# JuliaGaussianProcesses/ApproximateGPs.jl

Measured on NVIDIA B200. Metric: SVGP ELBO+grad points/sec (FP64), higher is better.
Workload: dtype f64

## Files before the change

### approximategps.jl_b200/csrc/agp.cu

```cuda
#include <dlfcn.h>
#include <nccl.h>
#include <stdarg.h>
#include <stdio.h>
#include <string.h>

#include <algorithm>
#include <string>
#include <vector>

#include "../../include/agp.h"
#include "dense.cuh"
#include "f32sweep.cuh"
#include "gemm.cuh"
#include "kfun.cuh"
#include "laplace.cuh"
#include "sweep.cuh"

using namespace agp;

static thread_local std::string g_err;
static thread_local int32_t g_err_info = 0;
static int32_t fail(int32_t code, const char* fmt, ...) {
  char buf[1024];
  va_list ap;
// ... 87 lines not shown
  LikParams lp;
  std::vector<double> h_m;
};

enum { PC_TRSM_FWD = 0, PC_GEMM_BTA, PC_PERPOINT, PC_GEMM_BC, PC_TRSM_BWD, PC_SYRK, PC_KGRAD, PC_PREPARE, PC_FINISH, PC_ALLREDUCE, PC_LAPLACE, PC_F32_AUX, PC_COUNT };
static const char* const kProfNames[PC_COUNT] = {"trsm_kuf_fwd", "gemm_BtA", "perpoint", "gemm_BC", "trsm_bwd", "syrk_G", "kgrad",
                                                 "prepare_step", "finish_epilogue", "allreduce", "laplace", "f32_planes_gvec"};
struct ProfRec {
  int cls;
  cudaEvent_t a, b;
};
struct Prof {
  bool on = false;
  std::vector<cudaEvent_t> pool;
  size_t used = 0;
  std::vector<ProfRec> recs;
  double ms[PC_COUNT] = {0};
  int64_t cnt[PC_COUNT] = {0};
  cudaEvent_t get() {
    if (used == pool.size()) {
      cudaEvent_t e;
      cudaEventCreate(&e);
      pool.push_back(e);
    }
    return pool[used++];
  }
};

static void lap_release(agp_ctx* c);
static void chol_partition_release(agp_ctx* c);
struct agp_ctx {
  Prof prof;
  void* lap = nullptr;
  int device = 0;
  cudaStream_t stream = nullptr;
  cudaStream_t stream2 = nullptr;
  cudaEvent_t ev_trail = nullptr;
  cudaStream_t stream3 = nullptr;
  int part_state = 0;
  CUgreenCtx part_chain = nullptr, part_bulk = nullptr;
  cudaStream_t pstream_chain = nullptr, pstream_side = nullptr, pstream_trail = nullptr;
  cudaEvent_t ev_enter = nullptr, ev_leave = nullptr;
  int part_sms_chain = 0, part_sms_bulk = 0;
  cudaEvent_t ev_diag = nullptr, ev_prow = nullptr, ev_side = nullptr, ev_prio = nullptr;
  cudaStream_t stream_copy = nullptr;
  cudaEvent_t ev_copy = nullptr;
  int sms = 148;
  int64_t launches = 0;
  int64_t chunk_cols = 0;
  int nslab = 0, nsplit = 0;
  DevBuf z, zs, zn, zsp, mvec, mt, Lq, Kw, Lk, Lt, Ut, Bt_cm, Bt_rm, W1, W2, W3, W4, vec64, vec64b;
  DevBuf A, C, Ab, As, saa, sam, scc_part, dmu, dv, sc_part;
  DevBuf Kf, DKb;
  DevBuf gpart, Gpart, kpart, red, small, ghbuf;
  DevBuf qBt7, sBt7, sPm;
  DevBuf q6A, q6As, s6;
  DevBuf fA, fC, fAb, fAs, fBtc, fBtr, fLi;
  DevBuf qAb, sAb, qLi, sLi;
  DevBuf qK, sK, qLi7, sLi7, sxx_part;
  int* d_flags = nullptr;
  SvgpState st;
  ncclComm_t comm = nullptr;
  int nranks = 1, rank = 0;
  DevBuf mu_out, var_out, px1, px2, pxs1, pxn1, pxs2, pxn2, pcov;
};

struct agp_dataset {
  agp_ctx* ctx = nullptr;
  int64_t cap = 0, N = 0;
  int D = 0;
  double* X = nullptr;
  double* y = nullptr;
  DevBuf stage;
};

#define LAUNCHED(ctx) ((ctx)->launches++)
struct ProfScope {
  agp_ctx* c;
  bool on;
  ProfScope(agp_ctx* c_, int cls) : c(c_), on(c_->prof.on) {
    if (!on) return;
    ProfRec r{cls, c->prof.get(), c->prof.get()};
    cudaEventRecord(r.a, c->stream);
    c->prof.recs.push_back(r);
  }
  ~ProfScope() {
    if (on) cudaEventRecord(c->prof.recs.back().b, c->stream);
  }
};
#define KCHECK()                                                                                   \
  do {                                                                                             \
    cudaError_t e_ = cudaGetLastError();                                                           \
    if (e_ != cudaSuccess) return fail(AGP_ERR_CUDA, "kernel launch failed: %s (%s:%d)", cudaGetErrorString(e_), __FILE__, __LINE__); \
  } while (0)

extern "C" int32_t agp_ctx_create(int32_t device, agp_ctx** out) {
  if (!out) return fail(AGP_ERR_INVALID, "agp_ctx_create: out is NULL");
  int ndev = 0;
  cudaError_t e = cudaGetDeviceCount(&ndev);
  if (e != cudaSuccess || ndev == 0)
    return fail(AGP_ERR_CUDA, "no CUDA device available (%s); this library has no CPU fallback", cudaGetErrorString(e));
  if (device < 0 || device >= ndev) return fail(AGP_ERR_INVALID, "device %d out of range (0..%d)", device, ndev - 1);
  CU(cudaSetDevice(device));
  cudaDeviceProp prop;
  CU(cudaGetDeviceProperties(&prop, device));
  if (prop.major < 10)
    return fail(AGP_ERR_UNSUPPORTED, "device %s is sm_%d%d; this library is built for sm_100a only", prop.name, prop.major, prop.minor);
  agp_ctx* c = new agp_ctx();
  c->device = device;
  c->sms = prop.multiProcessorCount;
  int prio_lo = 0, prio_hi = 0;
  CU(cudaDeviceGetStreamPriorityRange(&prio_lo, &prio_hi));
  CU(cudaStreamCreateWithPriority(&c->stream, cudaStreamNonBlocking, prio_hi));
  CU(cudaStreamCreateWithPriority(&c->stream2, cudaStreamNonBlocking, prio_lo));
  CU(cudaStreamCreateWithPriority(&c->stream3, cudaStreamNonBlocking, prio_hi < prio_lo - 1 ? prio_hi + 1 : prio_hi));
  CU(cudaEventCreateWithFlags(&c->ev_trail, cudaEventDisableTiming));
  CU(cudaEventCreateWithFlags(&c->ev_diag, cudaEventDisableTiming));
  CU(cudaEventCreateWithFlags(&c->ev_prow, cudaEventDisableTiming));
  CU(cudaEventCreateWithFlags(&c->ev_side, cudaEventDisableTiming));
  CU(cudaEventCreateWithFlags(&c->ev_prio, cudaEventDisableTiming));
  CU(cudaStreamCreateWithFlags(&c->stream_copy, cudaStreamNonBlocking));
  CU(cudaEventCreateWithFlags(&c->ev_copy, cudaEventDisableTiming));
  CU(cudaMalloc(&c->d_flags, 4 * sizeof(int)));
  CU(cudaMemset(c->d_flags, 0, 4 * sizeof(int)));
  *out = c;
  return AGP_OK;
}

extern "C" int32_t agp_ctx_destroy(agp_ctx* c) {
  if (!c) return AGP_OK;
  cudaSetDevice(c->device);
  cudaStreamSynchronize(c->stream);
  if (c->comm && g_nccl.CommDestroy) g_nccl.CommDestroy(c->comm);
  DevBuf* bufs[] = {&c->z, &c->zs, &c->zn, &c->zsp, &c->mvec, &c->mt, &c->Lq, &c->Kw, &c->Lk, &c->Lt, &c->Ut, &c->Bt_cm, &c->Bt_rm,
                    &c->W1, &c->W2, &c->W3, &c->W4, &c->vec64, &c->vec64b, &c->A, &c->C, &c->Ab, &c->As, &c->Kf, &c->DKb, &c->saa, &c->sam,
                    &c->scc_part, &c->dmu, &c->dv, &c->sc_part, &c->gpart, &c->Gpart, &c->kpart, &c->red, &c->small, &c->ghbuf, &c->q6A, &c->q6As, &c->s6, &c->qBt7, &c->sBt7, &c->sPm, &c->fA, &c->fC, &c->fAb, &c->fAs, &c->fBtc, &c->fBtr, &c->fLi, &c->qAb, &c->sAb, &c->qLi, &c->sLi, &c->qK, &c->sK, &c->qLi7, &c->sLi7, &c->sxx_part,
                    &c->mu_out, &c->var_out, &c->px1, &c->px2, &c->pxs1, &c->pxn1, &c->pxs2, &c->pxn2, &c->pcov};
  for (DevBuf* b : bufs) b->release();
  lap_release(c);
  if (c->d_flags) cudaFree(c->d_flags);
  for (cudaEvent_t e : c->prof.pool) cudaEventDestroy(e);
  if (c->ev_trail) cudaEventDestroy(c->ev_trail);
  if (c->stream2) cudaStreamDestroy(c->stream2);
  for (cudaEvent_t e : {c->ev_diag, c->ev_prow, c->ev_side, c->ev_prio})
    if (e) cudaEventDestroy(e);
  if (c->stream3) cudaStreamDestroy(c->stream3);
  chol_partition_release(c);
  if (c->ev_copy) cudaEventDestroy(c->ev_copy);
  if (c->stream_copy) cudaStreamDestroy(c->stream_copy);
  cudaStreamDestroy(c->stream);
  delete c;
  return AGP_OK;
}

extern "C" int32_t agp_ctx_stream(agp_ctx* c, void** s) {
  if (!c || !s) return fail(AGP_ERR_INVALID, "agp_ctx_stream: NULL argument");
  *s = (void*)c->stream;
  return AGP_OK;
}
extern "C" int32_t agp_ctx_profile(agp_ctx* c, int32_t enable) {
  if (!c) return fail(AGP_ERR_INVALID, "agp_ctx_profile: NULL");
  c->prof.on = enable != 0;
  return AGP_OK;
}
extern "C" const char* agp_profile_class_name(int32_t cls) { return (cls >= 0 && cls < PC_COUNT) ? kProfNames[cls] : nullptr; }
extern "C" int32_t agp_ctx_profile_read(agp_ctx* c, int32_t max_classes, double* ms_out, int64_t* count_out, int32_t* n_classes) {
  if (!c) return fail(AGP_ERR_INVALID, "agp_ctx_profile_read: NULL");
  CU(cudaSetDevice(c->device));
  CU(cudaStreamSynchronize(c->stream));
  Prof& p = c->prof;
  for (const ProfRec& r : p.recs) {
    float ms = 0.f;
    if (cudaEventElapsedTime(&ms, r.a, r.b) == cudaSuccess) {
      p.ms[r.cls] += ms;
      p.cnt[r.cls]++;
    }
  }
  p.recs.clear();
  p.used = 0;
  for (int i = 0; i < PC_COUNT && i < max_classes; i++) {
    if (ms_out) ms_out[i] = p.ms[i];
    if (count_out) count_out[i] = p.cnt[i];
  }
  if (n_classes) *n_classes = PC_COUNT;
  for (int i = 0; i < PC_COUNT; i++) {
    p.ms[i] = 0;
    p.cnt[i] = 0;
  }
// ... 138 lines not shown
  agp_ctx* c = ds->ctx;
  CU(cudaSetDevice(c->device));
  const int D = ds->D;
  if (ldx <= 0) ldx = layout == AGP_POINT_MAJOR ? D : N;
  const int64_t nflt = layout == AGP_POINT_MAJOR ? N * ldx : (int64_t)D * ldx;
  const float* src = X;
  if (location == AGP_HOST && N > 0) {
    OK(ds->stage.ensure((nflt + 1) / 2 + 1));
    CU(cudaMemcpyAsync(ds->stage.p, X, sizeof(float) * nflt, cudaMemcpyHostToDevice, c->stream));
    src = reinterpret_cast<const float*>(ds->stage.p);
  }
  if (N > 0) {
    widen_x_kernel<<<1024, 256, 0, c->stream>>>(src, ldx, layout, ds->X, N, D);
    LAUNCHED(c);
    KCHECK();
  }
  CU(cudaStreamSynchronize(c->stream));
  OK(upload_y(ds, y, N, ytype, location));
  CU(cudaStreamSynchronize(c->stream));
  ds->N = N;
  return AGP_OK;
}

extern "C" int32_t agp_dataset_size(agp_dataset* ds, int64_t* N, int32_t* D) {
  if (!ds) return fail(AGP_ERR_INVALID, "agp_dataset_size: NULL");
  if (N) *N = ds->N;
  if (D) *D = ds->D;
  return AGP_OK;
}
extern "C" int32_t agp_dataset_destroy(agp_dataset* ds) {
  if (!ds) return AGP_OK;
  cudaSetDevice(ds->ctx->device);
  if (ds->X) cudaFree(ds->X);
  if (ds->y) cudaFree(ds->y);
  ds->stage.release();
  delete ds;
  return AGP_OK;
}

template <auto Kernel>
static int32_t ensure_smem(agp_ctx* c, int bytes) {
  static int granted[64] = {0};
  int& g = granted[c->device & 63];
  if (g > bytes) return AGP_OK;
  if (bytes > 0) CU(cudaFuncSetAttribute(Kernel, cudaFuncAttributeMaxDynamicSharedMemorySize, bytes));
  g = bytes + 1;
  return AGP_OK;
}

template <int MODE, int S>
static int32_t launch_trsm_s(agp_ctx* c, const TrsmArgs& a, int tiles_n) {
  using Cfg = StageCfg<A_KM, B_KN>;
  const int Sx = (MODE == TR_KUF_FWD || MODE == TR_KUF_FWD_SCALED) ? kuf_dp(a.kp.D) + 2 : 0;
  const int smem = (S * (Cfg::elems + BK * Sx) + 64 * Sx) * 8 + 16;
  OK((ensure_smem<trsm_kernel<MODE, S>>(c, smem)));
  trsm_kernel<MODE, S><<<tiles_n, NTHREADS, smem, c->stream>>>(a);
  LAUNCHED(c);
  KCHECK();
  return AGP_OK;
}
template <int MODE>
static int32_t launch_trsm(agp_ctx* c, const TrsmArgs& a, int tiles_n);
static bool s1_fused() {
  static const bool fused = getenv("AGP_S1_FUSED") && atoi(getenv("AGP_S1_FUSED")) != 0;
  return fused;
}
static int32_t launch_s1(agp_ctx* c, const TrsmArgs& t1_in, int tiles_n, bool keep = false, bool gen_only = false) {
  if (s1_fused() && !gen_only) return launch_trsm<TR_KUF_FWD>(c, t1_in, tiles_n);
  TrsmArgs t1 = t1_in;
  KufGenArgs g{};
  g.K = keep ? c->Kf.p : t1.X;
  g.DK = (keep && t1.kp.kind != AGP_KERNEL_SE) ? c->DKb.p : nullptr;
  if (keep) t1.RHS = c->Kf.p;
  g.ldx = t1.ldx;
  g.ncols = tiles_n * BN;
  g.pts = t1.pts;
  g.npts = t1.npts;
  g.zsp = t1.zsp;
  g.kp = t1.kp;
  const int D = t1.kp.D;
  const int smem = 0;
  const dim3 grid((g.ncols + KG_COLS - 1) / KG_COLS, t1.nb * BM / KG_ROWS);
#define AGP_KGEN_D(KD)                                                                   \
  {                                                                                      \
    if (D <= 4) kuf_gen_kernel<4, KD><<<grid, KG_COLS, smem, c->stream>>>(g);            \
    else if (D <= 8) kuf_gen_kernel<8, KD><<<grid, KG_COLS, smem, c->stream>>>(g);       \
    else if (D <= 16) kuf_gen_kernel<16, KD><<<grid, KG_COLS, smem, c->stream>>>(g);     \
    else kuf_gen_kernel<32, KD><<<grid, KG_COLS, smem, c->stream>>>(g);                  \
  }
  switch (t1.kp.kind) {
    case AGP_KERNEL_SE: AGP_KGEN_D(AGP_KERNEL_SE) break;
    case AGP_KERNEL_MATERN32: AGP_KGEN_D(AGP_KERNEL_MATERN32) break;
    case AGP_KERNEL_MATERN52: AGP_KGEN_D(AGP_KERNEL_MATERN52) break;
    case AGP_KERNEL_LINEAR: AGP_KGEN_D(AGP_KERNEL_LINEAR) break;
    default: AGP_KGEN_D(AGP_KERNEL_SUM) break;
  }
#undef AGP_KGEN_D
  LAUNCHED(c);
  KCHECK();
  if (gen_only) return AGP_OK;
  return launch_trsm<TR_RHS_FWD_SUMS>(c, t1, tiles_n);
}

template <int MODE>
static int32_t launch_trsm(agp_ctx* c, const TrsmArgs& a, int tiles_n) {
  if ((MODE == TR_KUF_FWD || MODE == TR_KUF_FWD_SCALED) && a.kp.D > 8) return launch_trsm_s<MODE, 3>(c, a, tiles_n);
  return launch_trsm_s<MODE, 4>(c, a, tiles_n);
// ... 618 lines not shown
    theta = round_up(dZ + (int64_t)Mp * D, 16);
    total = theta + theta_size(D);
  }
};

static bool kgrad_fast(const SvgpState& st) {
  return !s1_fused() && st.kp.kind >= AGP_KERNEL_SE && st.kp.kind <= AGP_KERNEL_MATERN52;
}
static int64_t pick_chunk_cols(agp_ctx* c, int64_t count) {
  const int64_t wave = (int64_t)c->sms * 2 * BN;
  const int64_t by_mem = (int64_t)12e9 / (6 * 8 * std::max(c->st.Mp, BM)) / wave;
  int64_t cap = std::min<int64_t>(8, std::max<int64_t>(2, by_mem)) * wave;
  if (const char* e = getenv("AGP_CHUNK_COLS")) cap = std::max<int64_t>(BN, round_up(atoll(e), BN));
  return std::min<int64_t>(cap, round_up(std::max<int64_t>(count, 1), 2 * BN));
}

static int32_t ensure_sweep_workspace(agp_ctx* c, int64_t cols, bool grad) {
  const SvgpState& st = c->st;
  const int Mp = st.Mp, D = st.D, nb = st.nb;
  const int64_t MM = (int64_t)Mp * Mp;
  if (cols > c->chunk_cols) c->chunk_cols = cols;
  const int64_t cc = c->chunk_cols;
  OK(c->A.ensure((int64_t)Mp * cc));
  OK(c->C.ensure((int64_t)Mp * cc));
  OK(c->saa.ensure(cc));
  OK(c->sam.ensure(cc));
  OK(c->scc_part.ensure((int64_t)(st.f64_emu ? 4 : 2) * nb * cc));
  OK(c->dmu.ensure(cc));
  OK(c->dv.ensure(cc));
  OK(c->sc_part.ensure((cc / 256 + 2) * NSC));
  OK(c->red.ensure(RedLayout(Mp, D).total));
  if (st.f32) {
    OK(c->fA.ensure((int64_t)Mp * cc));
    OK(c->fC.ensure((int64_t)Mp * cc));
    if (grad) {
      OK(c->fAb.ensure((int64_t)Mp * cc));
      OK(c->fAs.ensure((int64_t)Mp * cc));
      OK(c->qAb.ensure(((int64_t)i8e::S5_NS * Mp * cc + 7) / 8));
      OK(c->sAb.ensure(2 * cc));
    }
  }
  if (st.f32 && Mp >= 768) {
    OK(c->Kf.ensure((int64_t)Mp * cc));
    OK(c->qK.ensure(((int64_t)i8e::S * Mp * cc + 7) / 8));
    OK(c->sK.ensure(cc));
    OK(c->sxx_part.ensure((int64_t)2 * (Mp / 32) * cc));
  }
  if (grad) {
    OK(c->Ab.ensure((int64_t)Mp * cc));
    OK(c->As.ensure((int64_t)Mp * cc));
    if (kgrad_fast(st)) {
      OK(c->Kf.ensure((int64_t)Mp * cc));
      if (st.kp.kind != AGP_KERNEL_SE) OK(c->DKb.ensure((int64_t)Mp * cc));
    }
    OK(c->gpart.ensure((cc / BN) * Mp));
    const int ntiles = nb * (nb + 1);
    const int by_waves = (8 * 2 * c->sms + ntiles - 1) / ntiles;
    const int by_mem = (int)std::max<int64_t>(1, ((int64_t)512 << 20) / (MM * 8));
    c->nsplit = std::max(1, std::min(std::min(by_waves, by_mem), 32));
    if (st.f64_emu && !st.f32) c->nsplit = std::max<int>(c->nsplit, (int)((round_up(cc, 128) + 16383) / 16384));
    OK(c->Gpart.ensure((int64_t)c->nsplit * MM));
    c->nslab = (int)std::max<int64_t>((cc + 2047) / 2048, (Mp + 2047) / 2048);
    OK(c->kpart.ensure((int64_t)c->nslab * Mp * kgrad_stride(D)));
    DevBuf* w[] = {&c->W1, &c->W2, &c->W3, &c->W4};
    for (DevBuf* b : w) OK(b->ensure(MM));
  }
  return AGP_OK;
}

static int32_t run_kgrad(agp_ctx* c, const double* Kb, int64_t ld, const double* pts, int npts, int nslab, const double* Kf = nullptr,
                         const double* DK = nullptr) {
  const SvgpState& st = c->st;
  KgradArgs a{};
  a.Kb = Kb;
  a.Kf = Kf;
  a.DK = DK;
  a.ld = ld;
  a.pts = pts;
  a.npts = npts;
  a.zs = c->zs.p;
  a.zn = c->zn.p;
  a.slab = 2048;
  a.part = c->kpart.p;
  a.stride = kgrad_stride(st.D);
  a.Mp = st.Mp;
  a.kp = st.kp;
  const dim3 grid((st.M + 7) / 8, nslab);
  if (Kf) {
    const bool se = st.kp.kind == AGP_KERNEL_SE;
#define AGP_KSTREAM(DM)                                                                              \
  {                                                                                                  \
    const int sm = KfTile<DM>::value * (DM + 2) * 8;                                                 \
    if (se) {                                                                                        \
      OK((ensure_smem<kgrad_stream_kernel<DM, true>>(c, sm)));                                       \
      kgrad_stream_kernel<DM, true><<<grid, 256, sm, c->stream>>>(a);                                \
    } else {                                                                                         \
      OK((ensure_smem<kgrad_stream_kernel<DM, false>>(c, sm)));                                      \
      kgrad_stream_kernel<DM, false><<<grid, 256, sm, c->stream>>>(a);                               \
    }                                                                                                \
  }
    if (st.D <= 4) AGP_KSTREAM(4)
    else if (st.D <= 8) AGP_KSTREAM(8)
    else if (st.D <= 16) AGP_KSTREAM(16)
    else AGP_KSTREAM(32)
#undef AGP_KSTREAM
    LAUNCHED(c);
// ... 232 lines not shown
      }
      if (s5t) {
        ProfScope ps(c, PC_TRSM_BWD);
        t5::EpiF5 e5{c->Ab.p, ldc};
        t5::Args g{Mp, t5::KM_FROM_N, 0, 0, t5::MnDesc()};
        OK((launch_t5<false, false>(c, grid5, fAb, plane, Mp, ncols, reinterpret_cast<float*>(c->fLi.p), MMf, Mp, Mp, g, e5)));
      } else {
        ProfScope ps(c, PC_TRSM_BWD);
        signed char* qAb = reinterpret_cast<signed char*>(c->qAb.p);
        const int64_t pbytes = (int64_t)Mp * ldc;
        i8e::transpose_slice_kernel<i8e::S5_NS><<<(ncols + 31) / 32, 256, 0, c->stream>>>(c->Ab.p, ldc, Mp, ncols, qAb, Mp, pbytes, c->sAb.p, c->sAb.p + ldc);
        LAUNCHED(c);
        KCHECK();
        CUtensorMap ma, mb;
        if (!i8e::make_map3(&ma, qAb, Mp, ncols, Mp, pbytes, i8e::EM, i8e::S5_NS) ||
            !i8e::make_map3(&mb, reinterpret_cast<signed char*>(c->qLi.p), Mp, Mp, Mp, MM, i8e::S5_N, i8e::S5_NS))
          return fail(AGP_ERR_CUDA, "cuTensorMapEncodeTiled failed");
        i8e::EpiE5 e5{c->Ab.p, ldc, c->sAb.p, c->sLi.p};
        i8e::Args g8{Mp, i8e::KM_FROM_N, 0, 0};
        constexpr int sm8 = i8e::Cfg<i8e::S5_NS, i8e::S5_N>::smem_bytes;
        OK((ensure_smem<i8e::i8emu_gemm_kernel<i8e::EpiE5, i8e::S5_NS, i8e::S5_N>>(c, sm8)));
        i8e::i8emu_gemm_kernel<i8e::EpiE5, i8e::S5_NS, i8e::S5_N><<<dim3(Mp / i8e::S5_N, ncols / i8e::EM, 1), i8e::E_THREADS, sm8, c->stream>>>(ma, mb, g8, e5);
        LAUNCHED(c);
        KCHECK();
      }
      {
        ProfScope ps(c, PC_SYRK);
        const int kchunk = (int)round_up((ncols + c->nsplit - 1) / c->nsplit, t5::TM);
        const int nz = (ncols + kchunk - 1) / kchunk;
        t5::EpiF6 e6{c->Gpart.p, Mp};
        t5::Args g{ncols, t5::KM_SPLIT, kchunk, 1, t5::MnDesc()};
        OK((launch_t5<true, true>(c, dim3(Mp / t5::TM, Mp / t5::TN, nz), fAs, plane, Mp, ncols, fA, plane, Mp, ncols, g, e6)));
      }
      {
        ProfScope ps(c, PC_F32_AUX);
        const int slab = 512, nslab = (ncols + slab - 1) / slab;
        t5::gvec_kernel<<<dim3((Mp / 4 + 255) / 256, nslab), 256, 0, c->stream>>>(fA, fA + plane, Mp, Mp, c->dmu.p, ncols, slab, c->gpart.p, Mp);
        LAUNCHED(c);
        KCHECK();
      }
    } else {
    EpiS4 e4{c->A.p, c->Ab.p, c->As.p, ldc, c->dmu.p, c->dv.p, c->mt.p, c->gpart.p, Mp};
    {
      ProfScope ps(c, PC_GEMM_BC);
      OK((run_gemm<A_KM, B_KN>(c, nb, tiles_n, c->Bt_cm.p, Mp, c->C.p, ldc, Mp, KR_LOWER, TS_ALL, e4)));
    }
    TrsmArgs t5a{};
    t5a.T = c->Ut.p;
    t5a.ldt = Mp;
    t5a.nb = nb;
    t5a.X = c->Ab.p;
    t5a.ldx = ldc;
    t5a.kp = st.kp;
    {
      ProfScope ps(c, PC_TRSM_BWD);
      OK(launch_trsm<TR_RHS_BWD>(c, t5a, tiles_n));
    }
    if (st.f64_emu && Mp >= 768 && ncols >= 2048) {
      ProfScope ps(c, PC_SYRK);
      const int64_t ldk = round_up(ncols, 128), pbytes = (int64_t)Mp * ldk;
      OK(c->q6A.ensure(((int64_t)i8e::S * pbytes + 7) / 8));
      OK(c->q6As.ensure(((int64_t)i8e::S * pbytes + 7) / 8));
      OK(c->s6.ensure(4 * (int64_t)Mp));
      double* sA = c->s6.p;
      double* sAs = c->s6.p + Mp;
      unsigned long long* mx = reinterpret_cast<unsigned long long*>(c->s6.p + 2 * Mp);
      CU(cudaMemsetAsync(mx, 0, sizeof(unsigned long long) * 2 * Mp, c->stream));
      const int seg = 8192;
      const dim3 gmx((ncols + seg - 1) / seg, Mp / 8);
      i8e::rowmax_kernel<<<gmx, 256, 0, c->stream>>>(c->A.p, ldc, Mp, ncols, seg, mx);
      i8e::rowmax_kernel<<<gmx, 256, 0, c->stream>>>(c->As.p, ldc, Mp, ncols, seg, mx + Mp);
      signed char* qA = reinterpret_cast<signed char*>(c->q6A.p);
      signed char* qAs = reinterpret_cast<signed char*>(c->q6As.p);
      const dim3 gsl((unsigned)((ldk + 1023) / 1024), Mp);
      i8e::slice_rows2d_kernel<i8e::S><<<gsl, 256, 0, c->stream>>>(c->A.p, ldc, ncols, qA, ldk, pbytes, mx, sA);
      i8e::slice_rows2d_kernel<i8e::S><<<gsl, 256, 0, c->stream>>>(c->As.p, ldc, ncols, qAs, ldk, pbytes, mx + Mp, sAs);
      c->launches += 4;
      KCHECK();
      CUtensorMap ma, mb;
      if (!i8e::make_map3(&ma, qAs, ldk, Mp, ldk, pbytes, i8e::EM, i8e::S) || !i8e::make_map3(&mb, qA, ldk, Mp, ldk, pbytes, i8e::EN, i8e::S))
        return fail(AGP_ERR_CUDA, "cuTensorMapEncodeTiled failed");
      const int kchunk = 16384, nz = (int)((ldk + kchunk - 1) / kchunk);
      if (nz > c->nsplit) return fail(AGP_ERR_ALLOC, "S6 (INT8): %d slabs of G needed, %d allocated", nz, c->nsplit);
      i8e::EpiE6 e6{c->Gpart.p, Mp, sAs, sA};
      i8e::Args g8{(int)ldk, i8e::KM_SPLIT, kchunk, 1};
      OK((ensure_smem<i8e::i8emu_gemm_kernel<i8e::EpiE6>>(c, i8e::SMEM_BYTES)));
      i8e::i8emu_gemm_kernel<i8e::EpiE6><<<dim3(Mp / i8e::EN, Mp / i8e::EM, nz), i8e::E_THREADS, i8e::SMEM_BYTES, c->stream>>>(ma, mb, g8, e6);
      LAUNCHED(c);
      KCHECK();
    } else {
      ProfScope ps(c, PC_SYRK);
      SyrkArgs s{};
      s.As = c->As.p;
      s.A = c->A.p;
      s.ld = ldc;
      s.ncols = ncols;
      s.kchunk = (int)round_up((ncols + c->nsplit - 1) / c->nsplit, BK);
      s.G = c->Gpart.p;
      s.Mp = Mp;
      using Cfg = StageCfg<A_MK, B_NK>;
      OK((ensure_smem<syrk_kernel>(c, Cfg::smem_bytes)));
      dim3 grid(nb * (nb + 1), c->nsplit);
      syrk_kernel<<<grid, NTHREADS, Cfg::smem_bytes, c->stream>>>(s);
      LAUNCHED(c);
      KCHECK();
    }
    }
    {
      ProfScope ps(c, PC_KGRAD);
      if (kgrad_fast(st)) {
        OK(run_kgrad(c, c->Ab.p, ldc, pts, npts, (npts + 2047) / 2048, c->Kf.p, st.kp.kind != AGP_KERNEL_SE ? c->DKb.p : nullptr));
      } else {
        OK(run_kgrad(c, c->Ab.p, ldc, pts, npts, (npts + 2047) / 2048));
      }
    }
  }
  if (predict || !grad) return AGP_OK;
  sum_slices_kernel<<<(Mp + 255) / 256, 256, 0, c->stream>>>(c->gpart.p, (int)(ldc / BN), Mp, Mp, c->red.p + rl.g);
  LAUNCHED(c);
  KCHECK();
  sum_slices_kernel<<<1024, 256, 0, c->stream>>>(c->Gpart.p, c->nsplit, MM, MM, c->red.p + rl.G);
  LAUNCHED(c);
  KCHECK();
  OK(finish_kgrad(c, c->nslab, 1.0, c->red.p + rl.dZ, c->red.p + rl.theta));
  return AGP_OK;
}

static int32_t check_dataset(agp_ctx* c, agp_dataset* ds, int64_t offset, int64_t count, int D) {
  if (!c || !ds) return fail(AGP_ERR_INVALID, "NULL context or dataset");
  if (ds->ctx != c) return fail(AGP_ERR_INVALID, "dataset belongs to another context");
  if (ds->D != D) return fail(AGP_ERR_INVALID, "dataset dimension %d != params.D %d", ds->D, D);
  const int64_t min_count = (c->comm && c->nranks > 1) ? 0 : 1;
  if (offset < 0 || count < min_count || offset + count > ds->N)
    return fail(AGP_ERR_INVALID, "points [%lld, %lld) outside the dataset (N=%lld)", (long long)offset, (long long)(offset + count), (long long)ds->N);
  return AGP_OK;
}

extern "C" int32_t agp_svgp_sweep(agp_ctx* c, agp_dataset* ds, int64_t offset, int64_t count, const agp_svgp_params* p,
                                  double num_data, int64_t global_batch, int32_t want_grad) {
  if (!c || !p) return fail(AGP_ERR_INVALID, "agp_svgp_sweep: NULL argument");
  if (c->comm && c->nranks > 1 && global_batch <= 0)
    return fail(AGP_ERR_INVALID, "with a communicator attached global_batch (the batch size summed over all ranks) is required: "
                                 "num_data / count of one shard would scale the ELBO by the number of ranks");
  OK(check_dataset(c, ds, offset, count, p->D));
  {
    ProfScope ps(c, PC_PREPARE);
    OK(prepare_step(c, p));
  }
  SvgpState& st = c->st;
  const int64_t gb = global_batch > 0 ? global_batch : count;
  st.scale = (num_data > 0 ? num_data : (double)gb) / (double)gb;
  st.want_grad = want_grad;
  st.point_base = offset + ((long long)c->rank << 40);
  OK(sweep_points(c, ds->X + offset * ds->D, ds->y + offset, count, want_grad != 0, false, nullptr, nullptr));
  st.sweep_pending = true;
  return AGP_OK;
}

extern "C" int32_t agp_svgp_reduce_buffer(agp_ctx* c, void** dptr, int64_t* n) {
  if (!c || !c->st.valid || !c->st.sweep_pending) return fail(AGP_ERR_INVALID, "agp_svgp_reduce_buffer: no sweep pending");
  RedLayout rl(c->st.Mp, c->st.D);
// ... 508 lines not shown
```

### approximategps.jl_b200/csrc/sweep.cuh

```cuda
#pragma once
#include "gemm.cuh"
#include "kfun.cuh"

namespace agp {

constexpr int TR_KUF_FWD = 0, TR_RHS_FWD = 1, TR_RHS_BWD = 2, TR_KUF_FWD_SCALED = 3, TR_RHS_FWD_SUMS = 4;

struct TrsmArgs {
  const double* T;
  int64_t ldt;
  int nb;
  double* X;
  int64_t ldx;
  const double* RHS;
  const double* pts;
  int npts;
  const double* zsp;
  const double* mt;
  double* saa;
  double* sam;
  const double* rowscale;
  const double* dvec;
  double* skd;
  KernelParams kp;
};

struct StepIter {
  int J, q, kk, cnt, nb;
  bool fwd;
  __device__ __forceinline__ void init(bool f, int nb_) {
    fwd = f;
    nb = nb_;
    J = f ? 0 : nb_ - 1;
    q = 0;
    kk = 0;
    cnt = 1 + (f ? J : nb - 1 - J);
  }
  __device__ __forceinline__ bool is_diag() const { return q == 0; }
  __device__ __forceinline__ int src() const { return q == 0 ? J : (fwd ? q - 1 : nb - q); }
  __device__ __forceinline__ bool last_in_row() const { return q == cnt - 1 && kk == BM / BK - 1; }
  __device__ __forceinline__ void next() {
    if (++kk == BM / BK) {
      kk = 0;
      if (++q == cnt) {
        q = 0;
        J += fwd ? 1 : -1;
        cnt = 1 + (fwd ? J : nb - 1 - J);
      }
    }
  }
};

template <bool SCALED>
__device__ __forceinline__ void gen_kuf_tile(double* __restrict__ sB, const double* __restrict__ sZ, const double* __restrict__ xs, int row0,
                                             const KernelParams& kp, int warp, int lane, const double* rowscale, const double* dvec, double (&pkd)[2]) {
  const int g = lane >> 2, t = lane & 3;
  const int D = kp.D, kind = kp.kind, Dq = kuf_dp(D), Sx = Dq + 2;
  const int c0 = warp * 8 + 2 * t;
  const double* z0 = sZ + g * Sx;
  const double* z1 = z0 + 8 * Sx;
  const double* xa = xs + c0 * Sx;
  const double* xb = xa + Sx;
  double u[2][2];
  if (D == 1 && kind != AGP_KERNEL_LINEAR) {
    const double d00 = xa[0] - z0[0], d01 = xb[0] - z0[0], d10 = xa[0] - z1[0], d11 = xb[0] - z1[0];
    u[0][0] = d00 * d00;
    u[0][1] = d01 * d01;
    u[1][0] = d10 * d10;
    u[1][1] = d11 * d11;
  } else {
    double acc0[2] = {0.0, 0.0}, acc1[2] = {0.0, 0.0};
    const double* xf = xs + (warp * 8 + g) * Sx + t;
    for (int k = 0; k < Dq; k += 4) {
      const double b = xf[k];
      dmma884(acc0, z0[k + t], b);
      dmma884(acc1, z1[k + t], b);
    }
    const double xna = xa[Dq], xnb = xb[Dq], zn0 = z0[Dq], zn1 = z1[Dq];
    u[0][0] = u_from_dot(kind, xna, zn0, acc0[0]);
    u[0][1] = u_from_dot(kind, xnb, zn0, acc0[1]);
    u[1][0] = u_from_dot(kind, xna, zn1, acc1[0]);
    u[1][1] = u_from_dot(kind, xnb, zn1, acc1[1]);
  }
#pragma unroll
  for (int h = 0; h < 2; h++) {
    const int row = row0 + g + 8 * h;
    const bool valid = row < kp.M;
    double v0 = valid ? kp.variance * kappa_kp(kp, u[h][0]) : 0.0;
    double v1 = valid ? kp.variance * kappa_kp(kp, u[h][1]) : 0.0;
    if (SCALED) {
      const double dv = dvec[row], rsc = rowscale[row];
      pkd[0] = fma(v0, dv, pkd[0]);
      pkd[1] = fma(v1, dv, pkd[1]);
      v0 *= rsc;
      v1 *= rsc;
    }
    *reinterpret_cast<double2*>(sB + (g + 8 * h) * BTile<B_KN>::ld + c0) = make_double2(v0, v1);
  }
}

template <int MODE, int S>
__global__ void __launch_bounds__(NTHREADS, 2) trsm_kernel(TrsmArgs a) {
  extern __shared__ __align__(128) double smem[];
  using Cfg = StageCfg<A_KM, B_KN>;
  constexpr bool SCALED = MODE == TR_KUF_FWD_SCALED;
  constexpr bool FWD = MODE == TR_KUF_FWD || SCALED;
  constexpr bool SUMS = FWD || MODE == TR_RHS_FWD_SUMS;
  ThreadMap tm;
  const int tid = threadIdx.x;
  const int n0 = blockIdx.x * BN;
  const int Sx = FWD ? kuf_dp(a.kp.D) + 2 : 0;
  const int stage_elems = Cfg::elems + BK * Sx;
  double* xs = smem + S * stage_elems;
  uint64_t* bar = reinterpret_cast<uint64_t*>(xs + 64 * Sx);

  if (FWD) {
    const int D = a.kp.D, Dq = kuf_dp(D);
    const int nvalid = max(0, min(BN, a.npts - n0));
    double* raw = smem;
    const double* src = a.pts + (int64_t)n0 * D;
    const unsigned bytes = (unsigned)(nvalid * D * 8);
    const bool use_tma = nvalid > 0 && ((reinterpret_cast<uintptr_t>(src) & 15) == 0) && ((bytes & 15) == 0);
    if (tid == 0) {
      mbar_init(bar, 1);
      fence_barrier_init();
    }
    __syncthreads();
    if (use_tma) {
      if (tid == 0) {
        mbar_expect_tx(bar, bytes);
        tma_bulk_g2s(raw, src, bytes, bar);
      }
      mbar_wait(bar, 0);
    } else {
      for (int i = tid; i < nvalid * D; i += NTHREADS) raw[i] = src[i];
      __syncthreads();
    }
    if (tid < BN) {
      double nrm = 0.0;
      for (int d = 0; d < D; d++) {
        const double v = (tid < nvalid) ? raw[tid * D + d] * a.kp.s[d] : 0.0;
        xs[tid * Sx + d] = v;
        nrm = fma(v, v, nrm);
      }
      for (int d = D; d < Sx; d++) xs[tid * Sx + d] = 0.0;
      xs[tid * Sx + Dq] = nrm;
    }
    __syncthreads();
  }

  double pkd[2] = {0.0, 0.0};
  StepIter it_issue, it_cons, it_gen;
  it_issue.init(MODE != TR_RHS_BWD, a.nb);
  it_cons.init(MODE != TR_RHS_BWD, a.nb);
  it_gen.init(true, a.nb);
  const int total = (BM / BK) * a.nb * (a.nb + 1) / 2;

  ALoad<A_KM> la;
  BLoad<B_KN> lb;
  la.init(a.ldt, tid);
  lb.init(a.ldx, tid);
  auto issue = [&](int slot) {
    double* st = smem + slot * stage_elems;
    const int J = it_issue.J, L = it_issue.src(), kk = it_issue.kk;
    la.load(st, a.T + (int64_t)(L * BM + kk * BK) * a.ldt + J * BM);
    if (FWD && it_issue.is_diag()) {
      const double* zsrc = a.zsp + (int64_t)(J * BM + kk * BK) * Sx;
      for (int ch = tid; ch < BK * Sx / 2; ch += NTHREADS) cp_async16(st + Cfg::elems + ch * 2, zsrc + ch * 2);
    } else {
      const double* bsrc = (a.RHS != nullptr && it_issue.is_diag()) ? a.RHS : a.X;
      lb.load(st + Cfg::a_elems, bsrc + (int64_t)(L * BM + kk * BK) * a.ldx + n0);
    }
    it_issue.next();
  };
  auto gen = [&](int slot) {
    double* st = smem + slot * stage_elems;
    gen_kuf_tile<SCALED>(st + Cfg::a_elems, st + Cfg::elems, xs, it_gen.J * BM + it_gen.kk * BK, a.kp, tm.warp, tm.lane, a.rowscale, a.dvec, pkd);
  };

  Acc acc;
  acc_zero(acc);
  double caa = 0.0, cam = 0.0;

#pragma unroll
  for (int s = 0; s < S - 1; s++) {
    if (s < total) issue(s);
    cp_async_commit();
  }
  if (FWD) {
    cp_async_wait<S - 2>();
    __syncthreads();
    gen(0);
    it_gen.next();
  }
  for (int step = 0; step < total; step++) {
    if (FWD) cp_async_wait<(S >= 3 ? S - 3 : 0)>();
    else cp_async_wait<S - 2>();
    __syncthreads();
    if (step + S - 1 < total) issue((step + S - 1) % S);
    cp_async_commit();
    const double* st = smem + (step % S) * stage_elems;
    const bool active = !it_cons.is_diag() || ((MODE == TR_RHS_BWD) ? tm.tri_active_upper(it_cons.kk * BK) : tm.tri_active_lower(it_cons.kk * BK));
    if (active) mma_stage<A_KM, B_KN>(acc, st, st + Cfg::a_elems, tm);
    if (FWD) {
      if (step + 1 < total && it_gen.is_diag()) gen((step + 1) % S);
      it_gen.next();
    }
    if (it_cons.last_in_row()) {
      const int J = it_cons.J;
      double qa[8], qm[8];
#pragma unroll
      for (int c = 0; c < 8; c++) qa[c] = qm[c] = 0.0;
#pragma unroll
      for (int mi = 0; mi < 4; mi++) {
        const int row = J * BM + tm.row(mi);
        const double mtr = SUMS ? a.mt[row] : 0.0;
        double* xr = a.X + (int64_t)row * a.ldx + n0;
#pragma unroll
        for (int ni = 0; ni < 4; ni++) {
          const double v0 = acc[mi][ni][0], v1 = acc[mi][ni][1];
          *reinterpret_cast<double2*>(xr + tm.col(ni, 0)) = make_double2(v0, v1);
          if (SUMS) {
            qa[2 * ni] = fma(v0, v0, qa[2 * ni]);
            qa[2 * ni + 1] = fma(v1, v1, qa[2 * ni + 1]);
            qm[2 * ni] = fma(v0, mtr, qm[2 * ni]);
            qm[2 * ni + 1] = fma(v1, mtr, qm[2 * ni + 1]);
          }
        }
      }
      if (SUMS) {
        const bool b2 = tm.g & 4, b1 = tm.g & 2, b0 = tm.g & 1;
#pragma unroll
        for (int j = 0; j < 4; j++) {
          const double sa = b2 ? qa[j] : qa[j + 4], sm = b2 ? qm[j] : qm[j + 4];
          qa[j] = (b2 ? qa[j + 4] : qa[j]) + __shfl_xor_sync(0xffffffffu, sa, 16);
          qm[j] = (b2 ? qm[j + 4] : qm[j]) + __shfl_xor_sync(0xffffffffu, sm, 16);
        }
#pragma unroll
        for (int j = 0; j < 2; j++) {
          const double sa = b1 ? qa[j] : qa[j + 2], sm = b1 ? qm[j] : qm[j + 2];
          qa[j] = (b1 ? qa[j + 2] : qa[j]) + __shfl_xor_sync(0xffffffffu, sa, 8);
          qm[j] = (b1 ? qm[j + 2] : qm[j]) + __shfl_xor_sync(0xffffffffu, sm, 8);
        }
        {
          const double sa = b0 ? qa[0] : qa[1], sm = b0 ? qm[0] : qm[1];
          caa += (b0 ? qa[1] : qa[0]) + __shfl_xor_sync(0xffffffffu, sa, 4);
          cam += (b0 ? qm[1] : qm[0]) + __shfl_xor_sync(0xffffffffu, sm, 4);
        }
      }
      acc_zero(acc);
      __threadfence();
    }
    it_cons.next();
  }
  cp_async_wait<0>();
  if (SUMS) {
    __syncthreads();
    double* sred = smem;
    {
      const int col = tm.wn + (((tm.g >> 2) & 1) * 2 + ((tm.g >> 1) & 1)) * 8 + 2 * tm.t + (tm.g & 1);
      sred[(tm.wm >> 5) * 64 + col] = caa;
      sred[256 + (tm.wm >> 5) * 64 + col] = cam;
    }
    __syncthreads();
    if (tid < BN) {
      a.saa[n0 + tid] = ((sred[tid] + sred[64 + tid]) + sred[128 + tid]) + sred[192 + tid];
      a.sam[n0 + tid] = ((sred[256 + tid] + sred[320 + tid]) + sred[384 + tid]) + sred[448 + tid];
    }
    if (SCALED) {
#pragma unroll
      for (int e = 0; e < 2; e++) {
        double v = pkd[e];
#pragma unroll
        for (int o = 4; o < 32; o <<= 1) v += __shfl_xor_sync(0xffffffffu, v, o);
        if (tm.g == 0) a.skd[n0 + tm.warp * 8 + 2 * tm.t + e] = v;
      }
    }
  }
}

struct KufGenArgs {
  double* K;
  double* DK;
  int64_t ldx;
  int ncols;
  const double* pts;
  int npts;
  const double* zsp;
  KernelParams kp;
};
constexpr int KG_ROWS = 128, KG_COLS = 256;
template <int DMAX, int KIND>
__global__ void __launch_bounds__(KG_COLS) kuf_gen_kernel(KufGenArgs a) {
  constexpr int SZ = DMAX + 2;
  __shared__ __align__(16) double kgz[KG_ROWS * SZ];
  constexpr int kind = KIND;
  const int D = a.kp.D, Dq = kuf_dp(D), Sx = Dq + 2;
  const int row0 = blockIdx.y * KG_ROWS;
  const int n = blockIdx.x * KG_COLS + threadIdx.x;
  for (int i = threadIdx.x; i < KG_ROWS * SZ; i += KG_COLS) {
    const int r = i / SZ, d = i - r * SZ;
    const double* src = a.zsp + (int64_t)(row0 + r) * Sx;
    kgz[i] = d < D ? src[d] : (d == DMAX ? src[Dq] : 0.0);
  }
  double x[DMAX];
  double xn = 0.0;
#pragma unroll
  for (int d = 0; d < DMAX; d++) {
    x[d] = (d < D && n < a.npts) ? a.pts[(int64_t)n * D + d] * a.kp.s[d] : 0.0;
    xn = fma(x[d], x[d], xn);
  }
  __syncthreads();
  if (n >= a.ncols) return;
  const bool direct = D == 1 && kind != AGP_KERNEL_LINEAR;
  double* out = a.K + (int64_t)row0 * a.ldx + n;
  double* outd = a.DK ? a.DK + (int64_t)row0 * a.ldx + n : nullptr;
  const double var = a.kp.variance;
  const int rvalid = max(0, min(KG_ROWS, a.kp.M - row0));
  const double* z = kgz;
#pragma unroll 4
  for (int r = 0; r < rvalid; r++, z += SZ, out += a.ldx) {
    double u;
    if (direct) {
      const double df = x[0] - z[0];
      u = df * df;
    } else {
      double dot = 0.0;
#pragma unroll
      for (int d = 0; d < DMAX; d += 2) {
        const double2 zz = *reinterpret_cast<const double2*>(z + d);
        dot = fma(x[d], zz.x, dot);
// ... 486 lines not shown
        const bool ok = p < cnt;
        kb[buf][i] = ok ? kbr[t0 + p] : 0.0;
        kf[buf][i] = ok ? kfr[t0 + p] : 0.0;
        if (!SE) dk[buf][i] = ok ? dkr[t0 + p] : 0.0;
      }
    };
    fetch(0, 0);
    int buf = 0;
    for (int c0 = 0; c0 < cnt; c0 += 32 * U, buf ^= 1) {
      if (c0 + 32 * U < cnt) fetch(buf ^ 1, c0 + 32 * U);
#pragma unroll
      for (int i = 0; i < U; i++) {
        const double* xr = kf_smem + (c0 + lane + 32 * i) * Sx;
        const double kbv = kb[buf][i];
        dvar = fma(kbv, kf[buf][i], dvar);
        const double W = SE ? -0.5 * (kbv * kf[buf][i]) : kbv * dk[buf][i];
        rs += W;
#pragma unroll
        for (int d = 0; d < DMAX; d += 2) {
          const double2 v = *reinterpret_cast<const double2*>(xr + d);
          const double w0 = W * v.x, w1 = W * v.y;
          wx[d] += w0;
          wxx[d] = fma(w0, v.x, wxx[d]);
          wx[d + 1] += w1;
          wxx[d + 1] = fma(w1, v.y, wxx[d + 1]);
        }
      }
    }
  }
#pragma unroll
  for (int o = 16; o > 0; o >>= 1) {
    rs += __shfl_xor_sync(0xffffffffu, rs, o);
    dvar += __shfl_xor_sync(0xffffffffu, dvar, o);
#pragma unroll
    for (int d = 0; d < DMAX; d++) {
      wx[d] += __shfl_xor_sync(0xffffffffu, wx[d], o);
      wxx[d] += __shfl_xor_sync(0xffffffffu, wxx[d], o);
    }
  }
  if (lane == 0 && rvalid) {
    double* out = a.part + ((int64_t)slab * a.Mp + row) * a.stride;
    out[0] += rs;
    out[1] += dvar / a.kp.variance;
#pragma unroll
    for (int d = 0; d < DMAX; d++)
      if (d < D) {
        const double z = a.zs[(int64_t)row * D + d];
        out[3 + d] += wx[d];
        out[3 + D + d] += fma(z, fma(z, rs, -2.0 * wx[d]), wxx[d]);
      }
  }
}

struct KgradFinishArgs {
  const double* part;
  int nslab;
  int Mp;
  int stride;
  const double* zs;
  double zfac;
  double* dZ;
  double* theta;
  KernelParams kp;
};

__global__ void __launch_bounds__(256) kgrad_finish_kernel(KgradFinishArgs a) {
  __shared__ double sred[8];
  const int D = a.kp.D;
  const bool linear = a.kp.kind == AGP_KERNEL_LINEAR;
  double tv = 0.0, tc = 0.0;
  for (int j = 0; j < 2 + D; j++) {
    double v = 0.0;
    for (int row = threadIdx.x; row < a.kp.M; row += blockDim.x) {
      double s = 0.0;
      for (int sl = 0; sl < a.nslab; sl++) {
        const double* in = a.part + ((int64_t)sl * a.Mp + row) * a.stride;
        s += (j == 0) ? in[1] : (j == 1) ? in[2] : in[3 + D + (j - 2)];
      }
      v += s;
    }
    const double r = block_sum(v, sred);
    if (threadIdx.x == 0) {
      if (j == 0) tv = r;
      else if (j == 1) tc = r;
      else {
        const int d = j - 2;
        a.theta[2 + d] += (a.kp.s[d] != 0.0) ? 2.0 / a.kp.s[d] * r : 0.0;
      }
    }
  }
  if (threadIdx.x == 0) {
    a.theta[0] += tv;
    a.theta[1] += linear ? a.kp.variance * tc : 0.0;
  }
  if (kernel_is_composite(a.kp.kind)) {
    for (int j = 0; j < 2 * MAXC; j++) {
      double v = 0.0;
      for (int row = threadIdx.x; row < a.kp.M; row += blockDim.x) {
        double s = 0.0;
        for (int sl = 0; sl < a.nslab; sl++) s += a.part[((int64_t)sl * a.Mp + row) * a.stride + 3 + 2 * D + j];
        v += s;
      }
      const double r = block_sum(v, sred);
      if (threadIdx.x == 0) {
        const int c = j % MAXC;
        a.theta[2 + D + j] += (j < MAXC) ? a.kp.variance * r : a.kp.variance * r * 2.0 * sqrt(a.kp.ca[c]);
// ... 19 lines not shown
```

Measured before the change: 5.483 million.

## Fuse kernel-gradient accumulation into backward TRSM tail with per-tile partials

```diff
diff --git a/approximategps.jl_b200/csrc/agp.cu b/approximategps.jl_b200/csrc/agp.cu
--- a/approximategps.jl_b200/csrc/agp.cu
+++ b/approximategps.jl_b200/csrc/agp.cu
@@ -163,6 +163,7 @@
   DevBuf z, zs, zn, zsp, mvec, mt, Lq, Kw, Lk, Lt, Ut, Bt_cm, Bt_rm, W1, W2, W3, W4, vec64, vec64b;
   DevBuf A, C, Ab, As, saa, sam, scc_part, dmu, dv, sc_part;
   DevBuf Kf, DKb;
+  DevBuf ktile;
   DevBuf gpart, Gpart, kpart, red, small, ghbuf;
   DevBuf qBt7, sBt7, sPm;
   DevBuf q6A, q6As, s6;
@@ -244,7 +245,7 @@
   cudaStreamSynchronize(c->stream);
   if (c->comm && g_nccl.CommDestroy) g_nccl.CommDestroy(c->comm);
   DevBuf* bufs[] = {&c->z, &c->zs, &c->zn, &c->zsp, &c->mvec, &c->mt, &c->Lq, &c->Kw, &c->Lk, &c->Lt, &c->Ut, &c->Bt_cm, &c->Bt_rm,
-                    &c->W1, &c->W2, &c->W3, &c->W4, &c->vec64, &c->vec64b, &c->A, &c->C, &c->Ab, &c->As, &c->Kf, &c->DKb, &c->saa, &c->sam,
+                    &c->W1, &c->W2, &c->W3, &c->W4, &c->vec64, &c->vec64b, &c->A, &c->C, &c->Ab, &c->As, &c->Kf, &c->DKb, &c->ktile, &c->saa, &c->sam,
                     &c->scc_part, &c->dmu, &c->dv, &c->sc_part, &c->gpart, &c->Gpart, &c->kpart, &c->red, &c->small, &c->ghbuf, &c->q6A, &c->q6As, &c->s6, &c->qBt7, &c->sBt7, &c->sPm, &c->fA, &c->fC, &c->fAb, &c->fAs, &c->fBtc, &c->fBtr, &c->fLi, &c->qAb, &c->sAb, &c->qLi, &c->sLi, &c->qK, &c->sK, &c->qLi7, &c->sLi7, &c->sxx_part,
                     &c->mu_out, &c->var_out, &c->px1, &c->px2, &c->pxs1, &c->pxn1, &c->pxs2, &c->pxn2, &c->pcov};
   for (DevBuf* b : bufs) b->release();
@@ -489,7 +490,8 @@
 static int32_t launch_trsm_s(agp_ctx* c, const TrsmArgs& a, int tiles_n) {
   using Cfg = StageCfg<A_KM, B_KN>;
   const int Sx = (MODE == TR_KUF_FWD || MODE == TR_KUF_FWD_SCALED) ? kuf_dp(a.kp.D) + 2 : 0;
-  const int smem = (S * (Cfg::elems + BK * Sx) + 64 * Sx) * 8 + 16;
+  int smem = (S * (Cfg::elems + BK * Sx) + 64 * Sx) * 8 + 16;
+  if (MODE == TR_RHS_BWD_KGRAD) smem = std::max(smem, kt_smem_bytes(a.kp.D));
   OK((ensure_smem<trsm_kernel<MODE, S>>(c, smem)));
   trsm_kernel<MODE, S><<<tiles_n, NTHREADS, smem, c->stream>>>(a);
   LAUNCHED(c);
@@ -1214,6 +1216,7 @@
     if (kgrad_fast(st)) {
       OK(c->Kf.ensure((int64_t)Mp * cc));
       if (st.kp.kind != AGP_KERNEL_SE) OK(c->DKb.ensure((int64_t)Mp * cc));
+      if (!st.f32) OK(c->ktile.ensure((round_up(cc, 2 * BN) / BN) * Mp * kt_q(D)));
     }
     OK(c->gpart.ensure((cc / BN) * Mp));
     const int ntiles = nb * (nb + 1);
@@ -1552,7 +1555,21 @@
     t5a.X = c->Ab.p;
     t5a.ldx = ldc;
     t5a.kp = st.kp;
-    {
+    if (kgrad_fast(st)) {
+      ProfScope ps(c, PC_TRSM_BWD);
+      t5a.pts = pts;
+      t5a.npts = npts;
+      t5a.Kf = c->Kf.p;
+      t5a.DK = st.kp.kind != AGP_KERNEL_SE ? c->DKb.p : nullptr;
+      t5a.ktile = c->ktile.p;
+      OK(launch_trsm<TR_RHS_BWD_KGRAD>(c, t5a, tiles_n));
+      const int nslab = (npts + 2047) / 2048;
+      const int64_t nthr = (int64_t)nslab * st.M * D;
+      kgrad_tile_reduce_kernel<<<(unsigned)((nthr + 255) / 256), 256, 0, c->stream>>>(c->ktile.p, tiles_n, nslab, Mp, c->zs.p, c->kpart.p,
+                                                                                     kgrad_stride(D), st.kp);
+      LAUNCHED(c);
+      KCHECK();
+    } else {
       ProfScope ps(c, PC_TRSM_BWD);
       OK(launch_trsm<TR_RHS_BWD>(c, t5a, tiles_n));
     }
@@ -1606,7 +1623,7 @@
       KCHECK();
     }
     }
-    {
+    if (st.f32 || !kgrad_fast(st)) {
       ProfScope ps(c, PC_KGRAD);
       if (kgrad_fast(st)) {
         OK(run_kgrad(c, c->Ab.p, ldc, pts, npts, (npts + 2047) / 2048, c->Kf.p, st.kp.kind != AGP_KERNEL_SE ? c->DKb.p : nullptr));
diff --git a/approximategps.jl_b200/csrc/sweep.cuh b/approximategps.jl_b200/csrc/sweep.cuh
--- a/approximategps.jl_b200/csrc/sweep.cuh
+++ b/approximategps.jl_b200/csrc/sweep.cuh
@@ -4,7 +4,7 @@
 
 namespace agp {
 
-constexpr int TR_KUF_FWD = 0, TR_RHS_FWD = 1, TR_RHS_BWD = 2, TR_KUF_FWD_SCALED = 3, TR_RHS_FWD_SUMS = 4;
+constexpr int TR_KUF_FWD = 0, TR_RHS_FWD = 1, TR_RHS_BWD = 2, TR_KUF_FWD_SCALED = 3, TR_RHS_FWD_SUMS = 4, TR_RHS_BWD_KGRAD = 5;
 
 struct TrsmArgs {
   const double* T;
@@ -23,6 +23,9 @@
   const double* dvec;
   double* skd;
   KernelParams kp;
+  const double* Kf;
+  const double* DK;
+  double* ktile;
 };
 
 struct StepIter {
@@ -99,6 +102,132 @@
   }
 }
 
+__device__ __forceinline__ void stage_point_tile(double* raw, const double* src, int nvalid, int D, uint64_t* bar) {
+  const int tid = threadIdx.x;
+  const unsigned bytes = (unsigned)(nvalid * D * 8);
+  const bool use_tma = nvalid > 0 && ((reinterpret_cast<uintptr_t>(src) & 15) == 0) && ((bytes & 15) == 0);
+  if (tid == 0) {
+    mbar_init(bar, 1);
+    fence_barrier_init();
+  }
+  __syncthreads();
+  if (use_tma) {
+    if (tid == 0) {
+      mbar_expect_tx(bar, bytes);
+      tma_bulk_g2s(raw, src, bytes, bar);
+    }
+    mbar_wait(bar, 0);
+  } else {
+    for (int i = tid; i < nvalid * D; i += NTHREADS) raw[i] = src[i];
+    __syncthreads();
+  }
+}
+
+constexpr int KT_ROWS = 64, KT_LD = BN + PAD;
+__host__ __device__ __forceinline__ int kt_q(int D) { return 2 + 2 * D; }
+__host__ __device__ __forceinline__ int kt_ntiles(int D) { return (2 * D + 7) / 8; }
+__host__ __device__ __forceinline__ int kt_ldy(int D) { return 8 * kt_ntiles(D) + PAD; }
+__host__ __device__ __forceinline__ int kt_smem_bytes(int D) { return (2 * KT_ROWS * KT_LD + BN * kt_ldy(D)) * 8 + 16; }
+
+template <int R, bool MAT>
+__device__ __forceinline__ void kt_fill_chunk(const double* __restrict__ X, const double* __restrict__ Kf, const double* __restrict__ DK, int64_t ldx,
+                                              int n0, int c, int nvalid, int M, int r0, int warp, double* sW, double* sV) {
+#pragma unroll 1
+  for (int h = 0; h < KT_ROWS / (8 * R); h++) {
+    double2 kb[R], kf[R], dk[MAT ? R : 1];
+#pragma unroll
+    for (int i = 0; i < R; i++) {
+      const int64_t off = (int64_t)(r0 + (R * h + i) * 8 + warp) * ldx + n0 + c;
+      kb[i] = *reinterpret_cast<const double2*>(X + off);
+      kf[i] = *reinterpret_cast<const double2*>(Kf + off);
+      if (MAT) dk[i] = *reinterpret_cast<const double2*>(DK + off);
+    }
+#pragma unroll
+    for (int i = 0; i < R; i++) {
+      const int r = (R * h + i) * 8 + warp;
+      const bool rok = r0 + r < M;
+      const bool ok0 = rok && c < nvalid, ok1 = rok && c + 1 < nvalid;
+      const double2 v = make_double2(ok0 ? kb[i].x * kf[i].x : 0.0, ok1 ? kb[i].y * kf[i].y : 0.0);
+      if (MAT) {
+        *reinterpret_cast<double2*>(sW + r * KT_LD + c) = make_double2(ok0 ? kb[i].x * dk[i].x : 0.0, ok1 ? kb[i].y * dk[i].y : 0.0);
+        *reinterpret_cast<double2*>(sV + r * KT_LD + c) = v;
+      } else {
+        *reinterpret_cast<double2*>(sW + r * KT_LD + c) = v;
+      }
+    }
+  }
+}
+
+__device__ __noinline__ void kgrad_tail_rows(const double* __restrict__ X, const double* __restrict__ Kf, const double* __restrict__ DK,
+                                             double* __restrict__ ktile, int64_t ldx, int n0, int nvalid, int M, int Mp, int D, double* smem) {
+  constexpr int NTMAX = (2 * MAXD + 7) / 8;
+  const int warp = threadIdx.x >> 5, lane = threadIdx.x & 31, g = lane >> 2, t = lane & 3;
+  const int ntr = kt_ntiles(D), ldy = kt_ldy(D), Q = kt_q(D);
+  const bool se = DK == nullptr;
+  double* sW = smem;
+  double* sV = sW + KT_ROWS * KT_LD;
+  const double* sY = sV + KT_ROWS * KT_LD;
+  const double e0 = g == 0 ? 1.0 : 0.0, e1 = g == 1 ? 1.0 : 0.0;
+  const double sc = se ? -0.5 : 1.0;
+  const int c = 2 * lane;
+  for (int r0 = 0; r0 < M; r0 += KT_ROWS) {
+    if (se) kt_fill_chunk<8, false>(X, Kf, DK, ldx, n0, c, nvalid, M, r0, warp, sW, sV);
+    else kt_fill_chunk<4, true>(X, Kf, DK, ldx, n0, c, nvalid, M, r0, warp, sW, sV);
+    __syncthreads();
+    double acc[NTMAX][2], accs[2] = {0.0, 0.0};
+#pragma unroll
+    for (int nt = 0; nt < NTMAX; nt++) acc[nt][0] = acc[nt][1] = 0.0;
+    const double* aw = sW + (8 * warp + g) * KT_LD + t;
+    const double* av = sV + (8 * warp + g) * KT_LD + t;
+    const double* by = sY + t * ldy + g;
+#pragma unroll 4
+    for (int k = 0; k < BN; k += 4) {
+      const double w = aw[k];
+      dmma884(accs, w, e0);
+      if (!se) dmma884(accs, av[k], e1);
+#pragma unroll
+      for (int nt = 0; nt < NTMAX; nt++)
+        if (nt < ntr) dmma884(acc[nt], w, by[k * ldy + 8 * nt]);
+    }
+    const int row = r0 + 8 * warp + g;
+    if (row < M) {
+      double* out = ktile + ((int64_t)blockIdx.x * Mp + row) * Q;
+      if (t == 0) *reinterpret_cast<double2*>(out) = make_double2(sc * accs[0], se ? accs[0] : accs[1]);
+#pragma unroll
+      for (int nt = 0; nt < NTMAX; nt++)
+#pragma unroll
+        for (int e = 0; e < 2; e++) {
+          const int j = 8 * nt + 2 * t + e;
+          if (nt < ntr && j < 2 * D) out[2 + j] = sc * acc[nt][e];
+        }
+    }
+    __syncthreads();
+  }
+}
+
+__device__ __forceinline__ void kgrad_tail(const TrsmArgs& a, double* smem, int n0) {
+  const int tid = threadIdx.x, D = a.kp.D, ldy = kt_ldy(D);
+  double* sW = smem;
+  double* sY = smem + 2 * KT_ROWS * KT_LD;
+  uint64_t* bar = reinterpret_cast<uint64_t*>(sY + BN * ldy);
+  const int nvalid = max(0, min(BN, a.npts - n0));
+  __syncthreads();
+  fence_proxy_async();
+  stage_point_tile(sW, a.pts + (int64_t)n0 * D, nvalid, D, bar);
+  for (int i = tid; i < BN * ldy; i += NTHREADS) {
+    const int p = i / ldy, j = i - p * ldy;
+    double v = 0.0;
+    if (p < nvalid && j < 2 * D) {
+      const int d = j < D ? j : j - D;
+      const double x = sW[p * D + d] * a.kp.s[d];
+      v = j < D ? x : x * x;
+    }
+    sY[i] = v;
+  }
+  __syncthreads();
+  kgrad_tail_rows(a.X, a.Kf, a.DK, a.ktile, a.ldx, n0, nvalid, a.kp.M, a.nb * BM, D, smem);
+}
+
 template <int MODE, int S>
 __global__ void __launch_bounds__(NTHREADS, 2) trsm_kernel(TrsmArgs a) {
   extern __shared__ __align__(128) double smem[];
@@ -106,6 +235,8 @@
   constexpr bool SCALED = MODE == TR_KUF_FWD_SCALED;
   constexpr bool FWD = MODE == TR_KUF_FWD || SCALED;
   constexpr bool SUMS = FWD || MODE == TR_RHS_FWD_SUMS;
+  constexpr bool KGRAD = MODE == TR_RHS_BWD_KGRAD;
+  constexpr bool BWD = MODE == TR_RHS_BWD || KGRAD;
   ThreadMap tm;
   const int tid = threadIdx.x;
   const int n0 = blockIdx.x * BN;
@@ -118,24 +249,7 @@
     const int D = a.kp.D, Dq = kuf_dp(D);
     const int nvalid = max(0, min(BN, a.npts - n0));
     double* raw = smem;
-    const double* src = a.pts + (int64_t)n0 * D;
-    const unsigned bytes = (unsigned)(nvalid * D * 8);
-    const bool use_tma = nvalid > 0 && ((reinterpret_cast<uintptr_t>(src) & 15) == 0) && ((bytes & 15) == 0);
-    if (tid == 0) {
-      mbar_init(bar, 1);
-      fence_barrier_init();
-    }
-    __syncthreads();
-    if (use_tma) {
-      if (tid == 0) {
-        mbar_expect_tx(bar, bytes);
-        tma_bulk_g2s(raw, src, bytes, bar);
-      }
-      mbar_wait(bar, 0);
-    } else {
-      for (int i = tid; i < nvalid * D; i += NTHREADS) raw[i] = src[i];
-      __syncthreads();
-    }
+    stage_point_tile(raw, a.pts + (int64_t)n0 * D, nvalid, D, bar);
     if (tid < BN) {
       double nrm = 0.0;
       for (int d = 0; d < D; d++) {
@@ -151,8 +265,8 @@
 
   double pkd[2] = {0.0, 0.0};
   StepIter it_issue, it_cons, it_gen;
-  it_issue.init(MODE != TR_RHS_BWD, a.nb);
-  it_cons.init(MODE != TR_RHS_BWD, a.nb);
+  it_issue.init(!BWD, a.nb);
+  it_cons.init(!BWD, a.nb);
   it_gen.init(true, a.nb);
   const int total = (BM / BK) * a.nb * (a.nb + 1) / 2;
 
@@ -200,7 +314,7 @@
     if (step + S - 1 < total) issue((step + S - 1) % S);
     cp_async_commit();
     const double* st = smem + (step % S) * stage_elems;
-    const bool active = !it_cons.is_diag() || ((MODE == TR_RHS_BWD) ? tm.tri_active_upper(it_cons.kk * BK) : tm.tri_active_lower(it_cons.kk * BK));
+    const bool active = !it_cons.is_diag() || (BWD ? tm.tri_active_upper(it_cons.kk * BK) : tm.tri_active_lower(it_cons.kk * BK));
     if (active) mma_stage<A_KM, B_KN>(acc, st, st + Cfg::a_elems, tm);
     if (FWD) {
       if (step + 1 < total && it_gen.is_diag()) gen((step + 1) % S);
@@ -277,6 +391,7 @@
       }
     }
   }
+  if (KGRAD) kgrad_tail(a, smem, n0);
 }
 
 struct KufGenArgs {
@@ -869,6 +984,34 @@
   }
 }
 
+constexpr int KT_SLAB_TILES = 2048 / BN;
+__global__ void __launch_bounds__(256) kgrad_tile_reduce_kernel(const double* __restrict__ ktile, int tiles, int nslab, int Mp, const double* __restrict__ zs,
+                                                                double* part, int stride, KernelParams kp) {
+  const int D = kp.D, M = kp.M, Q = kt_q(D);
+  const int64_t i = (int64_t)blockIdx.x * blockDim.x + threadIdx.x;
+  if (i >= (int64_t)nslab * M * D) return;
+  const int d = (int)(i % D);
+  const int row = (int)((i / D) % M);
+  const int slab = (int)(i / ((int64_t)D * M));
+  const int t1 = min(tiles, (slab + 1) * KT_SLAB_TILES);
+  double rs = 0.0, dvar = 0.0, wx = 0.0, wxx = 0.0;
+  for (int t = slab * KT_SLAB_TILES; t < t1; t++) {
+    const double* in = ktile + ((int64_t)t * Mp + row) * Q;
+    rs += in[0];
+    wx += in[2 + d];
+    wxx += in[2 + D + d];
+    if (d == 0) dvar += in[1];
+  }
+  double* out = part + ((int64_t)slab * Mp + row) * stride;
+  const double z = zs[(int64_t)row * D + d];
+  out[3 + d] += wx;
+  out[3 + D + d] += fma(z, fma(z, rs, -2.0 * wx), wxx);
+  if (d == 0) {
+    out[0] += rs;
+    out[1] += dvar / kp.variance;
+  }
+}
+
 struct KgradFinishArgs {
   const double* part;
   int nslab;
```

Result: slower. 5.405 million (median of 6 runs) (-1.4%).
